# mirams/PyHillFit

Hardware: AMD Instinct MI355X
Metric: MCMC samples/sec (whole node) (higher is better)
Workload: dtype f64

## Files before the change

### pyhillfit_amd/csrc/phf_model.h

```cpp
#ifndef PHF_MODEL_H
#define PHF_MODEL_H

#include "phf_math.h"
#include "phf_philox.h"

#define PHF_SIGMA_FLOOR 1e-3
#define PHF_PIC50_RATE 0.2
#define PHF_PIC50_LOWER (-3.0)
#define PHF_HILL_UPPER 10.0
#define PHF_SIGMA_LOC 1e-3
#define PHF_SIGMA_SHAPE_M1 4.0
#define PHF_SIGMA_INV_SCALE (4.0 / (6.0 - 1e-3))
#define PHF_HILL_ARG_CAP 40.0

PHF_HD double phf_hill_den(int model, double ln_conc, double hill, double ln_ic50, phf_ktab k_exp) {
  const double a = (model == 1) ? (ln_conc - ln_ic50) : hill * (ln_conc - ln_ic50);
  return 1.0 + phf_exp_capped_k(__builtin_fmin(a, PHF_HILL_ARG_CAP), k_exp);
}

PHF_HD double phf_hill_percent(double w, phf_ktab k_exp) { return phf_fma(-PHF_K100(k_exp), w, PHF_K100(k_exp)); }
#define PHF_PCT_(w_) phf_hill_percent((w_), k_exp)

PHF_HD double phf_censored_z(double pred, double y, double inv_s) {
  const double sgn = (y > 50.0) ? 1.0 : -1.0;
  return (sgn * (pred - y)) * inv_s;
}

PHF_HD void phf_sl_log_target(int model, const double* lc, const double* y, const double* w, int n_other, int n_cens,
                              double n_other_points, double ss_within, double pi_bit, double temperature,
                              const double* th, phf_ktab k_exp, phf_ktab k_log,
                              double* out_lik, double* out_prior, double* out_ll1) {
  const double pic50 = th[0];
  const double hill = (model == 1) ? 1.0 : th[1];
  const double sigma = (model == 1) ? th[1] : th[2];
  const double ln_ic50 = PHF_LN10 * (6.0 - pic50);
  const double sl = sigma - PHF_SIGMA_LOC;
  const double inv_s = phf_rcp(sigma);
  const double log_sigma = phf_log_pos_k(sigma, k_log);
  const double log_sl = phf_log_pos_k(sl, k_log);

  double sse = ss_within, cens = 0.0;
  int j = 0;
  for (; j + 4 <= n_other; j += 4) {
    const phf_ktab ke = k_exp;
    const double d0 = phf_hill_den(model, lc[j], hill, ln_ic50, ke), d1 = phf_hill_den(model, lc[j + 1], hill, ln_ic50, ke);
    const double d2 = phf_hill_den(model, lc[j + 2], hill, ln_ic50, ke), d3 = phf_hill_den(model, lc[j + 3], hill, ln_ic50, ke);
    const double p01 = d0 * d1, p23 = d2 * d3;
    const double inv = phf_rcp(p01 * p23);
    const double i01 = inv * p23, i23 = inv * p01;
    const double r0 = y[j] - PHF_PCT_(i01 * d1), r1 = y[j + 1] - PHF_PCT_(i01 * d0);
    const double r2 = y[j + 2] - PHF_PCT_(i23 * d3), r3 = y[j + 3] - PHF_PCT_(i23 * d2);
    sse = phf_fma(w[j] * r0, r0, sse); sse = phf_fma(w[j + 1] * r1, r1, sse);
    sse = phf_fma(w[j + 2] * r2, r2, sse); sse = phf_fma(w[j + 3] * r3, r3, sse);
  }
  const int rem = n_other - j;
  if (rem == 3) {
    const phf_ktab ke = k_exp;
    const double d0 = phf_hill_den(model, lc[j], hill, ln_ic50, ke), d1 = phf_hill_den(model, lc[j + 1], hill, ln_ic50, ke);
    const double d2 = phf_hill_den(model, lc[j + 2], hill, ln_ic50, ke);
    const double p01 = d0 * d1;
    const double inv = phf_rcp(p01 * d2);
    const double i01 = inv * d2;
    const double r0 = y[j] - PHF_PCT_(i01 * d1), r1 = y[j + 1] - PHF_PCT_(i01 * d0);
    const double r2 = y[j + 2] - PHF_PCT_(inv * p01);
    sse = phf_fma(w[j] * r0, r0, sse); sse = phf_fma(w[j + 1] * r1, r1, sse); sse = phf_fma(w[j + 2] * r2, r2, sse);
  } else if (rem == 2) {
    const phf_ktab ke = k_exp;
    const double d0 = phf_hill_den(model, lc[j], hill, ln_ic50, ke), d1 = phf_hill_den(model, lc[j + 1], hill, ln_ic50, ke);
    const double inv = phf_rcp(d0 * d1);
    const double r0 = y[j] - PHF_PCT_(inv * d1), r1 = y[j + 1] - PHF_PCT_(inv * d0);
    sse = phf_fma(w[j] * r0, r0, sse); sse = phf_fma(w[j + 1] * r1, r1, sse);
  } else if (rem == 1) {
    const double r = y[j] - PHF_PCT_(phf_rcp(phf_hill_den(model, lc[j], hill, ln_ic50, k_exp)));
    sse = phf_fma(w[j] * r, r, sse);
  }
  j = n_other;
  const int n = n_other + n_cens;
  for (; j + 2 <= n; j += 2) {
    const phf_ktab ke = k_exp;
    const double d0 = phf_hill_den(model, lc[j], hill, ln_ic50, ke), d1 = phf_hill_den(model, lc[j + 1], hill, ln_ic50, ke);
    const double inv = phf_rcp(d0 * d1);
    const double z0 = phf_censored_z(PHF_PCT_(inv * d1), y[j], inv_s);
    const double z1 = phf_censored_z(PHF_PCT_(inv * d0), y[j + 1], inv_s);
    cens = phf_fma(w[j], phf_log_ndtr_tab(z0, -z0 * PHF_INV_SQRT2), cens);
    cens = phf_fma(w[j + 1], phf_log_ndtr_tab(z1, -z1 * PHF_INV_SQRT2), cens);
  }
  for (; j < n; ++j) {
    const double pred = PHF_PCT_(phf_rcp(phf_hill_den(model, lc[j], hill, ln_ic50, k_exp)));
    const double z = phf_censored_z(pred, y[j], inv_s);
    cens = phf_fma(w[j], phf_log_ndtr_tab(z, -z * PHF_INV_SQRT2), cens);
  }
  double a = cens - pi_bit;
  a = phf_fma(-n_other_points, log_sigma, a);
  a = phf_fma(-sse, 0.5 * inv_s * inv_s, a);
  if (sigma <= PHF_SIGMA_FLOOR) a = -PHF_INF;
  double lik = temperature * a;
  if (temperature == 0.0) lik = 0.0;
  *out_lik = lik;
  *out_ll1 = a;

  const int outside = (pic50 < PHF_PIC50_LOWER)
                      | (sigma <= PHF_SIGMA_LOC)
                      | ((model == 2) & ((hill < 0.0) | (hill > PHF_HILL_UPPER)));
  const double g = phf_fma(PHF_SIGMA_SHAPE_M1, log_sl, -sl * PHF_SIGMA_INV_SCALE);
  const double lp = -PHF_PIC50_RATE * pic50 + g;
  *out_prior = outside ? -PHF_INF : lp;
}

#define PHF_SHARE_PUT_(jj, d_) do { if (share_mask) den_slot[(jj) * slot_stride] = (d_); } while (0)
#define PHF_CDEN_(jj) ((((share_mask) >> ((jj) - n_other)) & 1u) ? den_slot[den_off[(jj) - n_other]] \
                                                                 : phf_hill_den(model, lc[jj], hill, ln_ic50, k_exp))
PHF_HD void phf_sl_log_target_shared(int model, const double* lc, const double* y, const double* w, int n_other, int n_cens,
                                     double n_other_points, double ss_within, double pi_bit, double temperature,
                                     const double* th, phf_ktab k_exp, phf_ktab k_log,
                                     unsigned share_mask, const int* den_off, double* den_slot, int slot_stride,
                                     double* out_lik, double* out_prior, double* out_ll1) {
  const double pic50 = th[0];
  const double hill = (model == 1) ? 1.0 : th[1];
  const double sigma = (model == 1) ? th[1] : th[2];
  const double ln_ic50 = PHF_LN10 * (6.0 - pic50);
  const double sl = sigma - PHF_SIGMA_LOC;
  const double inv_s = phf_rcp(sigma);
  const double log_sigma = phf_log_pos_k(sigma, k_log);
  const double log_sl = phf_log_pos_k(sl, k_log);

  double sse = ss_within, cens = 0.0;
  int j = 0;
  for (; j + 4 <= n_other; j += 4) {
    const phf_ktab ke = k_exp;
    const double d0 = phf_hill_den(model, lc[j], hill, ln_ic50, ke), d1 = phf_hill_den(model, lc[j + 1], hill, ln_ic50, ke);
    const double d2 = phf_hill_den(model, lc[j + 2], hill, ln_ic50, ke), d3 = phf_hill_den(model, lc[j + 3], hill, ln_ic50, ke);
    PHF_SHARE_PUT_(j, d0); PHF_SHARE_PUT_(j + 1, d1); PHF_SHARE_PUT_(j + 2, d2); PHF_SHARE_PUT_(j + 3, d3);
    const double p01 = d0 * d1, p23 = d2 * d3;
    const double inv = phf_rcp(p01 * p23);
    const double i01 = inv * p23, i23 = inv * p01;
    const double r0 = y[j] - PHF_PCT_(i01 * d1), r1 = y[j + 1] - PHF_PCT_(i01 * d0);
    const double r2 = y[j + 2] - PHF_PCT_(i23 * d3), r3 = y[j + 3] - PHF_PCT_(i23 * d2);
    sse = phf_fma(w[j] * r0, r0, sse); sse = phf_fma(w[j + 1] * r1, r1, sse);
    sse = phf_fma(w[j + 2] * r2, r2, sse); sse = phf_fma(w[j + 3] * r3, r3, sse);
  }
  const int rem = n_other - j;
  if (rem == 3) {
    const phf_ktab ke = k_exp;
    const double d0 = phf_hill_den(model, lc[j], hill, ln_ic50, ke), d1 = phf_hill_den(model, lc[j + 1], hill, ln_ic50, ke);
    const double d2 = phf_hill_den(model, lc[j + 2], hill, ln_ic50, ke);
    PHF_SHARE_PUT_(j, d0); PHF_SHARE_PUT_(j + 1, d1); PHF_SHARE_PUT_(j + 2, d2);
    const double p01 = d0 * d1;
    const double inv = phf_rcp(p01 * d2);
    const double i01 = inv * d2;
    const double r0 = y[j] - PHF_PCT_(i01 * d1), r1 = y[j + 1] - PHF_PCT_(i01 * d0);
    const double r2 = y[j + 2] - PHF_PCT_(inv * p01);
    sse = phf_fma(w[j] * r0, r0, sse); sse = phf_fma(w[j + 1] * r1, r1, sse); sse = phf_fma(w[j + 2] * r2, r2, sse);
  } else if (rem == 2) {
    const phf_ktab ke = k_exp;
    const double d0 = phf_hill_den(model, lc[j], hill, ln_ic50, ke), d1 = phf_hill_den(model, lc[j + 1], hill, ln_ic50, ke);
    PHF_SHARE_PUT_(j, d0); PHF_SHARE_PUT_(j + 1, d1);
    const double inv = phf_rcp(d0 * d1);
    const double r0 = y[j] - PHF_PCT_(inv * d1), r1 = y[j + 1] - PHF_PCT_(inv * d0);
    sse = phf_fma(w[j] * r0, r0, sse); sse = phf_fma(w[j + 1] * r1, r1, sse);
  } else if (rem == 1) {
    const double d0 = phf_hill_den(model, lc[j], hill, ln_ic50, k_exp);
    PHF_SHARE_PUT_(j, d0);
    const double r = y[j] - PHF_PCT_(phf_rcp(d0));
    sse = phf_fma(w[j] * r, r, sse);
  }
  j = n_other;
  const int n = n_other + n_cens;
  for (; j + 2 <= n; j += 2) {
    const double d0 = PHF_CDEN_(j), d1 = PHF_CDEN_(j + 1);
    const double inv = phf_rcp(d0 * d1);
    const double z0 = phf_censored_z(PHF_PCT_(inv * d1), y[j], inv_s);
    const double z1 = phf_censored_z(PHF_PCT_(inv * d0), y[j + 1], inv_s);
    cens = phf_fma(w[j], phf_log_ndtr_tab(z0, -z0 * PHF_INV_SQRT2), cens);
    cens = phf_fma(w[j + 1], phf_log_ndtr_tab(z1, -z1 * PHF_INV_SQRT2), cens);
  }
  for (; j < n; ++j) {
    const double pred = PHF_PCT_(phf_rcp(PHF_CDEN_(j)));
    const double z = phf_censored_z(pred, y[j], inv_s);
    cens = phf_fma(w[j], phf_log_ndtr_tab(z, -z * PHF_INV_SQRT2), cens);
  }
  double a = cens - pi_bit;
  a = phf_fma(-n_other_points, log_sigma, a);
  a = phf_fma(-sse, 0.5 * inv_s * inv_s, a);
  if (sigma <= PHF_SIGMA_FLOOR) a = -PHF_INF;
  double lik = temperature * a;
  if (temperature == 0.0) lik = 0.0;
  *out_lik = lik;
  *out_ll1 = a;

  const int outside = (pic50 < PHF_PIC50_LOWER)
                      | (sigma <= PHF_SIGMA_LOC)
                      | ((model == 2) & ((hill < 0.0) | (hill > PHF_HILL_UPPER)));
  const double g = phf_fma(PHF_SIGMA_SHAPE_M1, log_sl, -sl * PHF_SIGMA_INV_SCALE);
  const double lp = -PHF_PIC50_RATE * pic50 + g;
  *out_prior = outside ? -PHF_INF : lp;
}
#undef PHF_SHARE_PUT_
#undef PHF_CDEN_

PHF_HD double phf_sl_log_prior(int model, const double* th, phf_ktab k_log) {
  const double pic50 = th[0];
  const double hill = (model == 1) ? 1.0 : th[1];
  const double sigma = (model == 1) ? th[1] : th[2];
  const double sl = sigma - PHF_SIGMA_LOC;
  const double log_sl = phf_log_pos_k(sl, k_log);
  const int outside = (pic50 < PHF_PIC50_LOWER)
                      | (sigma <= PHF_SIGMA_LOC)
                      | ((model == 2) & ((hill < 0.0) | (hill > PHF_HILL_UPPER)));
  const double g = phf_fma(PHF_SIGMA_SHAPE_M1, log_sl, -sl * PHF_SIGMA_INV_SCALE);
  const double lp = -PHF_PIC50_RATE * pic50 + g;
  return outside ? -PHF_INF : lp;
}

PHF_HD double phf_mh_draws(int d, uint32_t chain_id, uint32_t problem_id, uint32_t t, uint32_t seed_lo,
                           uint32_t seed_hi, phf_ktab k_log, double* z) {
  const phf_u32x4 b = phf_philox_mh(chain_id, problem_id, t, 0u, seed_lo, seed_hi);
  z[0] = phf_normal_u32(b.w[0]);
  z[1] = phf_normal_u32(b.w[1]);
  if (d == 2) {
    z[2] = 0.0;
    const double u = phf_uniform53(b.w[2], b.w[3]);
    const double log_u = phf_log_pos_k(u, k_log);
    return (u < PHF_DBL_MIN) ? -PHF_INF : log_u;
  }
  z[2] = phf_normal_u32(b.w[2]);
  return phf_log_pos_k(phf_unit_open32(b.w[3]), k_log);
}

PHF_HD uint32_t phf_mh_draws_w3(uint32_t chain_id, uint32_t problem_id, uint32_t t, uint32_t seed_lo, uint32_t seed_hi, double* z) {
  const phf_u32x4 b = phf_philox_mh(chain_id, problem_id, t, 0u, seed_lo, seed_hi);
  z[0] = phf_normal_u32(b.w[0]);
  z[1] = phf_normal_u32(b.w[1]);
  z[2] = phf_normal_u32(b.w[2]);
  return b.w[3];
}

#define PHF_ACCEPT_U32_BAND 0x1p18f
PHF_HD int phf_mh_accept_u32(double x, uint32_t w, phf_ktab k_log) {
#if defined(__HIP_DEVICE_COMPILE__)
  const float t = __builtin_amdgcn_exp2f(__builtin_fmaf((float)x, 0x1.715476p+0f, 32.0f));
  const float dw = (float)w - t;
  bool acc = dw < 0.0f;
  if (PHF_ANY_LANE(__builtin_fabsf(dw) <= PHF_ACCEPT_U32_BAND)) {
    const bool exact = phf_log_pos_k(phf_unit_open32(w), k_log) < x;
    acc = (__builtin_fabsf(dw) <= PHF_ACCEPT_U32_BAND) ? exact : acc;
  }
  return acc;
#else
  return phf_log_pos_k(phf_unit_open32(w), k_log) < x;
#endif
}

#endif
```

### pyhillfit_amd/csrc/phf_philox.h

```cpp
#ifndef PHF_PHILOX_H
#define PHF_PHILOX_H

#include <stdint.h>

#if defined(__HIPCC__)
#define PHF_PHILOX_HD static __host__ __device__ __forceinline__
#else
#define PHF_PHILOX_HD static inline
#endif

typedef struct { uint32_t w[4]; } phf_u32x4;

#if defined(__HIP_DEVICE_COMPILE__)
#define PHF_XOR3(a, b, c) ((uint32_t)__builtin_amdgcn_bitop3_b32((int)(a), (int)(b), (int)(c), 0x96))
#else
#define PHF_XOR3(a, b, c) ((a) ^ (b) ^ (c))
#endif

#ifndef PHF_PHILOX_ROUNDS
#define PHF_PHILOX_ROUNDS 7
#endif

PHF_PHILOX_HD phf_u32x4 phf_philox4x32_r(int rounds, uint32_t c0, uint32_t c1, uint32_t c2, uint32_t c3,
                                         uint32_t k0, uint32_t k1) {
#if defined(__HIPCC__)
#pragma unroll
#endif
  for (int round = 0; round < rounds; ++round) {
    const uint64_t p0 = (uint64_t)0xD2511F53u * c0;
    const uint64_t p1 = (uint64_t)0xCD9E8D57u * c2;
    const uint32_t n0 = PHF_XOR3((uint32_t)(p1 >> 32), c1, k0);
    const uint32_t n2 = PHF_XOR3((uint32_t)(p0 >> 32), c3, k1);
    c1 = (uint32_t)p1; c3 = (uint32_t)p0; c0 = n0; c2 = n2;
    k0 += 0x9E3779B9u; k1 += 0xBB67AE85u;
  }
  phf_u32x4 out;
  out.w[0] = c0; out.w[1] = c1; out.w[2] = c2; out.w[3] = c3;
  return out;
}

PHF_PHILOX_HD phf_u32x4 phf_philox4x32_10(uint32_t c0, uint32_t c1, uint32_t c2, uint32_t c3, uint32_t k0, uint32_t k1) {
  return phf_philox4x32_r(10, c0, c1, c2, c3, k0, k1);
}
PHF_PHILOX_HD phf_u32x4 phf_philox4x32_7(uint32_t c0, uint32_t c1, uint32_t c2, uint32_t c3, uint32_t k0, uint32_t k1) {
  return phf_philox4x32_r(7, c0, c1, c2, c3, k0, k1);
}
PHF_PHILOX_HD phf_u32x4 phf_philox_mh(uint32_t c0, uint32_t c1, uint32_t c2, uint32_t c3, uint32_t k0, uint32_t k1) {
  return phf_philox4x32_r(PHF_PHILOX_ROUNDS, c0, c1, c2, c3, k0, k1);
}

#endif
```

### pyhillfit_amd/csrc/phf_single_level.hip

```cpp
#include <hip/hip_runtime.h>

#include "../../include/pyhillfit_amd.h"
#include "phf_common.h"
#include "phf_hier3_isa.h"
#include "phf_model.h"

namespace {

constexpr int kBlock = 64;
thread_local int g_last_sl_kernel = 0;
constexpr int kQueuePoison = 0x40000000;
constexpr int kQueueMaxRounds = 16;
constexpr int kDenSlots = 4;
constexpr int kMaxShared = 4;

template <int MODEL> struct Dim { static constexpr int d = (MODEL == 1) ? 2 : 3; };

#ifndef PHF_CHOL_FUSED_PIVOT
#define PHF_CHOL_FUSED_PIVOT 1
#endif
template <int D>
__device__ __forceinline__ void chol_packed(const double* c, double* l) {
  double inv[D];
#pragma unroll
  for (int i = 0; i < D; ++i) {
#pragma unroll
    for (int j = 0; j <= i; ++j) {
      double s = c[i * (i + 1) / 2 + j];
#pragma unroll
      for (int k = 0; k < j; ++k) s = phf_fma(-l[i * (i + 1) / 2 + k], l[j * (j + 1) / 2 + k], s);
      if (i == j) {
        const bool pos = s > 0.0;
        double ir = 0.0;
#if PHF_CHOL_FUSED_PIVOT
        const double rs = (i + 1 < D) ? phf_sqrt_rcp_pos(s, &ir) : phf_sqrt_pos(s);
#else
        const double rs = phf_sqrt_pos(s);
        ir = phf_rcp(rs);
#endif
        const double r = pos ? rs : 0.0;
        l[i * (i + 1) / 2 + i] = r;
        inv[i] = pos ? ir : 0.0;
      } else {
        l[i * (i + 1) / 2 + j] = s * inv[j];
      }
    }
  }
}

struct AdvanceArgs {
  phf_points pts;
  phf_problems prob;
  phf_mh_config cfg;
  int64_t t_begin, t_end;
  double* state;
  double* rows;
  double* moments;
  int64_t moments_after;
  int32_t blocks_per_problem;
  int32_t* queue;
  int32_t quantum;
  int32_t steady;
};

__device__ __forceinline__ void stage_points(const phf_points& pts, int pair, double* s_pts, int& n_other,
                                             int& n_zero, int& n_hundred) {
  const int32_t* cnt = pts.counts + 4 * pair;
  n_other = cnt[0]; n_zero = cnt[1]; n_hundred = cnt[2];
  const int n = n_other + n_zero + n_hundred;
  for (int j = threadIdx.x; j < n; j += kBlock) {
    s_pts[j] = pts.ln_conc[(size_t)pair * pts.stride + j];
    s_pts[pts.stride + j] = pts.response[(size_t)pair * pts.stride + j];
    s_pts[2 * pts.stride + j] = pts.weight[(size_t)pair * pts.stride + j];
  }
  __syncthreads();
}

template <int MODEL, bool MOMENTS, int KO, int KC, unsigned SHARE, bool LONE_WAVE, bool STEADY>
__device__ __forceinline__ void advance_body(const AdvanceArgs& a, const double* s_pts, double* s_den, const int* den_off, int q,
                                             int c, int pair, int n_other_rt, int n_cens_rt, const int64_t t_begin, const int64_t t_end) {
  static_assert(SHARE == 0 || (KO >= 1 && KO <= kDenSlots && KC >= 1 && KC <= kMaxShared && (SHARE >> KC) == 0),
                "shared denominators need a straight-line body with at most kDenSlots uncensored entries");
  constexpr int D = Dim<MODEL>::d;
  constexpr int NTRI = D * (D + 1) / 2;
  const int C = a.prob.chains_per_problem;
  const int n_other = (KO >= 0) ? KO : n_other_rt;
  const int n_cens = (KC >= 0) ? KC : n_cens_rt;
  const double* lc = s_pts;
  const double* yv = s_pts + a.pts.stride;
  const double* wv = s_pts + 2 * a.pts.stride;
  const double pi_bit = a.pts.pi_bit[pair];
  const double n_other_points = a.pts.extra[2 * pair], ss_within = a.pts.extra[2 * pair + 1];
  const double temperature = a.prob.temperature[q];
  const uint32_t pid = a.prob.problem_id[q];
  const uint32_t cid = a.prob.chain_id_base + (a.prob.chain_offset ? a.prob.chain_offset[q] : 0u) + (uint32_t)c;
  uint32_t seed_lo = (uint32_t)a.cfg.seed, seed_hi = (uint32_t)(a.cfg.seed >> 32);
  if (!LONE_WAVE) { asm volatile("" : "+v"(seed_lo)); asm volatile("" : "+v"(seed_hi)); }
  const size_t nchains = (size_t)a.prob.num_problems * C;
  const size_t g = (size_t)q * C + c;

  double th[D], mean[D], cov[NTRI], L[NTRI];
  double* sp = a.state + g;
#pragma unroll
  for (int i = 0; i < D; ++i) th[i] = sp[(size_t)i * nchains];
  double lt = sp[(size_t)D * nchains];
#pragma unroll
  for (int i = 0; i < D; ++i) mean[i] = sp[(size_t)(D + 1 + i) * nchains];
#pragma unroll
  for (int i = 0; i < NTRI; ++i) cov[i] = sp[(size_t)(2 * D + 1 + i) * nchains];
  double loga = sp[(size_t)(2 * D + 1 + NTRI) * nchains];
  const double nacc_in = sp[(size_t)(2 * D + 2 + NTRI) * nchains];
  uint32_t nacc = 0;
  double ll1 = sp[(size_t)(2 * D + 3 + NTRI) * nchains];
  PHF_KFETCH_V(k_exp, phf_k_exp, PHF_K_EXP_N);
  PHF_KFETCH_V(k_log, phf_k_log, PHF_K_LOG_N);
  chol_packed<D>(cov, L);
  double sc = phf_exp_fast_k(0.5 * loga, k_exp);

  double m1[D + 1], m2[D + 1], mll = 0.0;
  constexpr bool want_moments = MOMENTS;
  if (want_moments) {
#pragma unroll
    for (int i = 0; i <= D; ++i) {
      m1[i] = a.moments[(size_t)i * nchains + g];
      m2[i] = a.moments[(size_t)(D + 1 + i) * nchains + g];
    }
    mll = a.moments[(size_t)(2 * D + 2) * nchains + g];
  }

  const int thin = a.cfg.thinning;
  int until_save = thin - (int)(t_begin % thin);
  const bool save_rows = a.rows != nullptr;
  const size_t row_stride = (size_t)a.prob.num_problems * (D + 1) * C;
  double* out = a.rows + ((size_t)q * (D + 1)) * C + c + (size_t)(t_begin / thin - a.t_begin / thin) * row_stride;

  double z[3];
  double log_u = 0.0;
  uint32_t w_u = 0u;
  if constexpr (D == 3) w_u = phf_mh_draws_w3(cid, pid, (uint32_t)(t_begin + 1), seed_lo, seed_hi, z);
  else log_u = phf_mh_draws(D, cid, pid, (uint32_t)(t_begin + 1), seed_lo, seed_hi, k_log, z);
  const int64_t adapt_start = a.cfg.adapt_start;
  const bool adapt_in_range = adapt_start >= 0 && adapt_start <= 0xffffffffLL;
  const bool adapt_always = adapt_start < 0;
  const uint32_t adapt_at = adapt_start > 0xffffffffLL ? 0xffffffffu : (uint32_t)adapt_start;
  const bool reset_mean = a.cfg.reset_mean_at_adapt_start != 0 && adapt_in_range;
  const bool moments_always = a.moments_after < 0;
  const uint32_t moments_at = a.moments_after > 0xffffffffLL ? 0xffffffffu : (uint32_t)a.moments_after;
  int64_t gamma_i = t_begin + 1 - adapt_start;
  uint32_t t = (uint32_t)t_begin + 1u;
  for (uint32_t left = (uint32_t)(t_end - t_begin); left != 0; --left, ++t, ++gamma_i) {
    double star[D];
#pragma unroll
    for (int i = 0; i < D; ++i) {
      double v = L[i * (i + 1) / 2 + i] * z[i];
#pragma unroll
      for (int k = i - 1; k >= 0; --k) v = phf_fma(L[i * (i + 1) / 2 + k], z[k], v);
      star[i] = phf_fma(sc, v, th[i]);
    }
    double lik_star, prior_star, ll1_star;
    phf_sl_log_target_shared(MODEL, lc, yv, wv, n_other, n_cens, n_other_points, ss_within, pi_bit, temperature, star, k_exp, k_log,
                             SHARE, den_off, s_den + threadIdx.x, kBlock, &lik_star, &prior_star, &ll1_star);
    const double lt_star = lik_star + prior_star;
    const bool acc = (D == 3) ? (bool)phf_mh_accept_u32(lt_star - lt, w_u, k_log) : log_u < lt_star - lt;
    if (acc) {
#pragma unroll
      for (int i = 0; i < D; ++i) th[i] = star[i];
      lt = lt_star;
      ll1 = ll1_star;
    }
    nacc += acc ? 1u : 0u;
    double gs, gm, omg, omm;
    if constexpr (STEADY) {
      gs = a.cfg.gamma[gamma_i];
      omg = 1.0 - gs;
      gm = gs; omm = omg;
    } else {
      const bool adapting = adapt_always || t > adapt_at;
      const bool reset_now = reset_mean && t == adapt_at;
      const double gs_tab = a.cfg.gamma[adapting ? gamma_i : 0];
      gs = adapting ? gs_tab : 0.0;
      omg = 1.0 - gs;
      gm = reset_now ? 1.0 : gs; omm = reset_now ? 0.0 : omg;
    }
    {
      double v[D];
#pragma unroll
      for (int i = 0; i < D; ++i) v[i] = th[i] - mean[i];
#pragma unroll
      for (int i = 0; i < D; ++i)
#pragma unroll
        for (int j = 0; j <= i; ++j)
          cov[i * (i + 1) / 2 + j] = phf_fma(gs, v[i] * v[j], omg * cov[i * (i + 1) / 2 + j]);
#pragma unroll
      for (int i = 0; i < D; ++i) mean[i] = phf_fma(gm, th[i], omm * mean[i]);
      loga = phf_fma(gs, acc ? 0.75 : -0.25, loga);
    }
    double z_next[3];
    double log_u_next = 0.0;
    uint32_t w_u_next = 0u;
    if constexpr (D == 3) w_u_next = phf_mh_draws_w3(cid, pid, t + 1u, seed_lo, seed_hi, z_next);
    else log_u_next = phf_mh_draws(D, cid, pid, t + 1u, seed_lo, seed_hi, k_log, z_next);
    chol_packed<D>(cov, L);
    sc = phf_exp_fast_k(0.5 * loga, k_exp);
#pragma unroll
    for (int i = 0; i < 3; ++i) z[i] = z_next[i];
    log_u = log_u_next;
    w_u = w_u_next;
    if (--until_save == 0) {
      until_save = thin;
      if (save_rows) {
#pragma unroll
        for (int i = 0; i < D; ++i) out[(size_t)i * C] = th[i];
        out[(size_t)D * C] = lt;
        out += row_stride;
      }
      if (want_moments && (moments_always || t > moments_at)) {
#pragma unroll
        for (int i = 0; i < D; ++i) { m1[i] += th[i]; m2[i] = phf_fma(th[i], th[i], m2[i]); }
        m1[D] += lt; m2[D] = phf_fma(lt, lt, m2[D]);
        mll += ll1;
      }
    }
  }

#pragma unroll
  for (int i = 0; i < D; ++i) sp[(size_t)i * nchains] = th[i];
  sp[(size_t)D * nchains] = lt;
#pragma unroll
  for (int i = 0; i < D; ++i) sp[(size_t)(D + 1 + i) * nchains] = mean[i];
#pragma unroll
  for (int i = 0; i < NTRI; ++i) sp[(size_t)(2 * D + 1 + i) * nchains] = cov[i];
  sp[(size_t)(2 * D + 1 + NTRI) * nchains] = loga;
  sp[(size_t)(2 * D + 2 + NTRI) * nchains] = nacc_in + (double)nacc;
  sp[(size_t)(2 * D + 3 + NTRI) * nchains] = ll1;
  if (want_moments) {
#pragma unroll
    for (int i = 0; i <= D; ++i) {
      a.moments[(size_t)i * nchains + g] = m1[i];
      a.moments[(size_t)(D + 1 + i) * nchains + g] = m2[i];
    }
    a.moments[(size_t)(2 * D + 2) * nchains + g] = mll;
  }
}

#define PHF_BODY_(ko, kc, sh, steady) \
  advance_body<MODEL, MOMENTS, ko, kc, sh, WPS == 1, steady>(a, s_pts, s_den, den_off, q, c, pair, n_other, n_cens, t_from, t_to)
#define PHF_SHAPE_CASE(ko, kc) case (ko) * 8 + (kc): PHF_BODY_(ko, kc, 0u, true); break;
#define PHF_SHAPE_CASE_SHARED(ko, kc, sh) \
  case (ko) * 8 + (kc): if ((share & (sh)) == (sh)) PHF_BODY_(ko, kc, sh, true); else PHF_BODY_(ko, kc, 0u, true); break;
#define PHF_SHAPE_ROW(ko) PHF_SHAPE_CASE(ko, 0) PHF_SHAPE_CASE(ko, 1) PHF_SHAPE_CASE(ko, 2) PHF_SHAPE_CASE(ko, 3) PHF_SHAPE_CASE(ko, 4)

__device__ __forceinline__ unsigned share_map(const double* s_pts, int n_other, int n_cens, int* den_off) {
  unsigned share = 0;
#pragma unroll
  for (int m = 0; m < kMaxShared; ++m) {
    den_off[m] = 0;
    if (m < n_cens && n_other <= kDenSlots) {
      const long long b = __double_as_longlong(s_pts[n_other + m]);
#pragma unroll
      for (int j = kDenSlots - 1; j >= 0; --j)
        if (j < n_other && __double_as_longlong(s_pts[j]) == b) { share |= 1u << m; den_off[m] = j * kBlock; }
    }
    den_off[m] = __builtin_amdgcn_readfirstlane(den_off[m]);
  }
  return __builtin_amdgcn_readfirstlane(share);
}

template <int MODEL, bool MOMENTS, int WPS>
__device__ __forceinline__ void run_block(const AdvanceArgs& a, double* s_pts, double* s_den, int block, const int64_t t_begin,
                                          const int64_t t_end) {
  const int slot = block / a.blocks_per_problem;
  const int chunk = block - slot * a.blocks_per_problem;
  const int q = a.prob.launch_order ? a.prob.launch_order[slot] : slot;
  const int c = chunk * kBlock + threadIdx.x;
  int n_other, n_zero, n_hundred;
  const int pair = a.prob.pair_index[q];
  stage_points(a.pts, pair, s_pts, n_other, n_zero, n_hundred);
  if (c >= a.prob.chains_per_problem) return;
  const int n_cens = n_zero + n_hundred;
  int den_off[kMaxShared];
  const unsigned share = share_map(s_pts, n_other, n_cens, den_off);
  int64_t t_from = t_begin, t_to = t_end;
  if (a.steady == 0 || t_begin < a.cfg.adapt_start) {
    if (a.steady != 0 && a.cfg.adapt_start < t_end) t_to = a.cfg.adapt_start;
    PHF_BODY_(-1, -1, 0u, false);
    if (t_to == t_end) return;
    t_from = t_to; t_to = t_end;
  }
  if (n_other <= 5 && n_cens <= 4) {
    switch (n_other * 8 + n_cens) {
      PHF_SHAPE_CASE(0, 1) PHF_SHAPE_CASE(0, 2) PHF_SHAPE_CASE(0, 3) PHF_SHAPE_CASE(0, 4)
      PHF_SHAPE_CASE(1, 0) PHF_SHAPE_CASE(1, 1) PHF_SHAPE_CASE(1, 2) PHF_SHAPE_CASE(1, 3) PHF_SHAPE_CASE_SHARED(1, 4, 0x8u)
      PHF_SHAPE_CASE(2, 0) PHF_SHAPE_CASE_SHARED(2, 1, 0x1u) PHF_SHAPE_CASE_SHARED(2, 2, 0x3u) PHF_SHAPE_CASE_SHARED(2, 3, 0x4u)
      PHF_SHAPE_CASE_SHARED(2, 4, 0xcu)
      PHF_SHAPE_CASE(3, 0) PHF_SHAPE_CASE(3, 1) PHF_SHAPE_CASE_SHARED(3, 2, 0x2u) PHF_SHAPE_CASE_SHARED(3, 3, 0x6u)
      PHF_SHAPE_CASE_SHARED(3, 4, 0xeu)
      PHF_SHAPE_CASE(4, 0) PHF_SHAPE_CASE_SHARED(4, 1, 0x1u) PHF_SHAPE_CASE_SHARED(4, 2, 0x3u) PHF_SHAPE_CASE_SHARED(4, 3, 0x7u)
      PHF_SHAPE_CASE_SHARED(4, 4, 0xfu)
      PHF_SHAPE_ROW(5)
      default: PHF_BODY_(-1, -1, 0u, true); break;
    }
    return;
  }
  PHF_BODY_(-1, -1, 0u, true);
}

template <int MODEL, bool MOMENTS, int WPS>
__global__ __launch_bounds__(kBlock, WPS) void mh_advance_kernel(const AdvanceArgs a) {
  PHF_MATH_TABLES_TO_LDS();
  PHF_NORMAL_TABLE_TO_LDS();
  PHF_LOGPHI_TABLE_TO_LDS();
  extern __shared__ double s_pts[];
  __shared__ double s_den[kDenSlots * kBlock];
  const bool queued = a.queue != nullptr;
  const int nblocks = a.blocks_per_problem * a.prob.num_problems;
  const int total = queued ? nblocks * (int)((a.t_end - a.t_begin + a.quantum - 1) / a.quantum) : 0;
  for (;;) {
    int b = blockIdx.x, k = 0;
    int64_t t0 = a.t_begin, t1 = a.t_end;
    if (queued) {
      int task = 0;
      if (threadIdx.x == 0) task = atomicAdd(a.queue, 1);
      task = __builtin_amdgcn_readfirstlane(task);
      if (task >= total) break;
      k = task / nblocks; b = task - k * nblocks;
      if (k > 0) {
        int polls = 0;
        while (__hip_atomic_load(a.queue + 1 + b, __ATOMIC_RELAXED, __HIP_MEMORY_SCOPE_AGENT) < k) {
          __builtin_amdgcn_s_sleep(16);
          ++polls;
          const bool gave_up = polls > (1 << 24) ||
                               ((polls & 1023) == 0 && __hip_atomic_load(a.queue + 1 + nblocks, __ATOMIC_RELAXED, __HIP_MEMORY_SCOPE_AGENT) != 0);
          if (gave_up) {
            if (threadIdx.x == 0) {
              __hip_atomic_store(a.queue + 1 + nblocks, 1, __ATOMIC_RELAXED, __HIP_MEMORY_SCOPE_AGENT);
              __hip_atomic_store(a.queue, kQueuePoison, __ATOMIC_RELAXED, __HIP_MEMORY_SCOPE_AGENT);
            }
            return;
          }
        }
        __builtin_amdgcn_fence(__ATOMIC_ACQUIRE, "agent");
      }
      t0 = a.t_begin + (int64_t)k * a.quantum;
      t1 = (t0 + a.quantum < a.t_end) ? t0 + a.quantum : a.t_end;
    }
    run_block<MODEL, MOMENTS, WPS>(a, s_pts, s_den, b, t0, t1);
    if (!queued) break;
    __builtin_amdgcn_fence(__ATOMIC_RELEASE, "agent");
    asm volatile("s_waitcnt vmcnt(0)" ::: "memory");
    __syncthreads();
    if (threadIdx.x == 0) __hip_atomic_store(a.queue + 1 + b, k + 1, __ATOMIC_RELAXED, __HIP_MEMORY_SCOPE_AGENT);
  }
}

struct InitArgs {
  phf_points pts;
  phf_problems prob;
  int32_t cov_identity;
  double cov_scale;
  const double* theta0;
  double* state;
  double* row0;
  int32_t blocks_per_problem;
};

template <int MODEL>
__global__ __launch_bounds__(kBlock) void mh_init_kernel(const InitArgs a) {
  PHF_MATH_TABLES_TO_LDS();
  PHF_LOGPHI_TABLE_TO_LDS();
  constexpr int D = Dim<MODEL>::d;
  constexpr int NTRI = D * (D + 1) / 2;
  extern __shared__ double s_pts[];
  const int q = blockIdx.x / a.blocks_per_problem;
  const int chunk = blockIdx.x - q * a.blocks_per_problem;
  const int C = a.prob.chains_per_problem;
  const int c = chunk * kBlock + threadIdx.x;
  int n_other, n_zero, n_hundred;
  const int pair = a.prob.pair_index[q];
  stage_points(a.pts, pair, s_pts, n_other, n_zero, n_hundred);
  if (c >= C) return;
  const size_t nchains = (size_t)a.prob.num_problems * C;
  const size_t g = (size_t)q * C + c;
  double th[D];
#pragma unroll
  for (int i = 0; i < D; ++i) th[i] = a.theta0[(size_t)i * nchains + g];
  double lik0, prior0, ll10;
  PHF_KFETCH_V(k_exp, phf_k_exp, PHF_K_EXP_N);
  PHF_KFETCH_V(k_log, phf_k_log, PHF_K_LOG_N);
  phf_sl_log_target(MODEL, s_pts, s_pts + a.pts.stride, s_pts + 2 * a.pts.stride, n_other, n_zero + n_hundred,
                    a.pts.extra[2 * pair], a.pts.extra[2 * pair + 1], a.pts.pi_bit[pair], a.prob.temperature[q],
                    th, k_exp, k_log, &lik0, &prior0, &ll10);
  const double lt = lik0 + prior0;
  double* sp = a.state + g;
#pragma unroll
  for (int i = 0; i < D; ++i) { sp[(size_t)i * nchains] = th[i]; sp[(size_t)(D + 1 + i) * nchains] = th[i]; }
  sp[(size_t)D * nchains] = lt;
#pragma unroll
  for (int i = 0; i < D; ++i)
#pragma unroll
    for (int j = 0; j <= i; ++j)
      sp[(size_t)(2 * D + 1 + i * (i + 1) / 2 + j) * nchains] =
          (i != j) ? 0.0 : (a.cov_identity ? a.cov_scale : a.cov_scale * __builtin_fabs(th[i]));
  sp[(size_t)(2 * D + 1 + NTRI) * nchains] = 0.0;
  sp[(size_t)(2 * D + 2 + NTRI) * nchains] = 0.0;
  sp[(size_t)(2 * D + 3 + NTRI) * nchains] = ll10;
  if (a.row0) {
    double* o = a.row0 + ((size_t)q * (D + 1)) * C + c;
#pragma unroll
    for (int i = 0; i < D; ++i) o[(size_t)i * C] = th[i];
    o[(size_t)D * C] = lt;
  }
}

template <int MODEL>
__global__ __launch_bounds__(256) void log_target_kernel(const phf_points pts, int64_t m, const int32_t* pair_index,
                                                          const double* temperature, const double* theta,
                                                          double* out_lik, double* out_prior) {
  PHF_MATH_TABLES_TO_LDS();
  PHF_LOGPHI_TABLE_TO_LDS();
  constexpr int D = Dim<MODEL>::d;
  const int64_t i = (int64_t)blockIdx.x * 256 + threadIdx.x;
  if (i >= m) return;
  const int pair = pair_index[i];
  const int32_t* cnt = pts.counts + 4 * pair;
  double th[D];
#pragma unroll
  for (int k = 0; k < D; ++k) th[k] = theta[(size_t)k * m + i];
  double lik, prior, ll1;
  PHF_KFETCH_V(k_exp, phf_k_exp, PHF_K_EXP_N);
  PHF_KFETCH_V(k_log, phf_k_log, PHF_K_LOG_N);
  phf_sl_log_target(MODEL, pts.ln_conc + (size_t)pair * pts.stride, pts.response + (size_t)pair * pts.stride,
                    pts.weight + (size_t)pair * pts.stride, cnt[0], cnt[1] + cnt[2], pts.extra[2 * pair], pts.extra[2 * pair + 1],
                    pts.pi_bit[pair], temperature[i], th, k_exp, k_log, &lik, &prior, &ll1);
  if (out_lik) out_lik[i] = lik;
  if (out_prior) out_prior[i] = prior;
}

__global__ void debug_math_kernel(int fn, int64_t n, const double* in, double* out) {
  PHF_MATH_TABLES_TO_LDS();
  PHF_LOGPHI_TABLE_TO_LDS();
  PHF_ERFC_TABLE_TO_LDS();
  PHF_NORMAL_TABLE_TO_LDS();
// ... 227 lines not shown
```

Baseline: 73.47 billion.

## Split Philox rounds into lane-invariant and wave-uniform parts; drop redundant sigma floor

Precomputes the first two Philox rounds' per-chain (lane) contributions once, and computes the per-iteration part that depends only on problem id and step with wave-uniform (readfirstlane) values. Each step then only runs the remaining rounds, which cuts per-step VALU integer multiplies in the RNG. It also removes the likelihood's sigma floor check in the MH path, because the prior already returns -inf at the same bound (enforced by a static_assert). This relies on pid and t being wave-uniform and on the algebraic split exactly reproducing the original Philox stream.

```diff
diff --git a/pyhillfit_amd/csrc/phf_model.h b/pyhillfit_amd/csrc/phf_model.h
--- a/pyhillfit_amd/csrc/phf_model.h
+++ b/pyhillfit_amd/csrc/phf_model.h
@@ -110,11 +110,12 @@
 #define PHF_SHARE_PUT_(jj, d_) do { if (share_mask) den_slot[(jj) * slot_stride] = (d_); } while (0)
 #define PHF_CDEN_(jj) ((((share_mask) >> ((jj) - n_other)) & 1u) ? den_slot[den_off[(jj) - n_other]] \
                                                                  : phf_hill_den(model, lc[jj], hill, ln_ic50, k_exp))
-PHF_HD void phf_sl_log_target_shared(int model, const double* lc, const double* y, const double* w, int n_other, int n_cens,
-                                     double n_other_points, double ss_within, double pi_bit, double temperature,
-                                     const double* th, phf_ktab k_exp, phf_ktab k_log,
-                                     unsigned share_mask, const int* den_off, double* den_slot, int slot_stride,
-                                     double* out_lik, double* out_prior, double* out_ll1) {
+PHF_HD void phf_sl_log_target_shared_impl_(int model, const double* lc, const double* y, const double* w, int n_other, int n_cens,
+                                           double n_other_points, double ss_within, double pi_bit, double temperature,
+                                           const double* th, phf_ktab k_exp, phf_ktab k_log,
+                                           unsigned share_mask, const int* den_off, double* den_slot, int slot_stride,
+                                           int floor_select,
+                                           double* out_lik, double* out_prior, double* out_ll1) {
   const double pic50 = th[0];
   const double hill = (model == 1) ? 1.0 : th[1];
   const double sigma = (model == 1) ? th[1] : th[2];
@@ -182,7 +183,7 @@
   double a = cens - pi_bit;
   a = phf_fma(-n_other_points, log_sigma, a);
   a = phf_fma(-sse, 0.5 * inv_s * inv_s, a);
-  if (sigma <= PHF_SIGMA_FLOOR) a = -PHF_INF;
+  if (floor_select && sigma <= PHF_SIGMA_FLOOR) a = -PHF_INF;
   double lik = temperature * a;
   if (temperature == 0.0) lik = 0.0;
   *out_lik = lik;
@@ -197,6 +198,29 @@
 }
 #undef PHF_SHARE_PUT_
 #undef PHF_CDEN_
+
+PHF_HD void phf_sl_log_target_shared(int model, const double* lc, const double* y, const double* w, int n_other, int n_cens,
+                                     double n_other_points, double ss_within, double pi_bit, double temperature,
+                                     const double* th, phf_ktab k_exp, phf_ktab k_log,
+                                     unsigned share_mask, const int* den_off, double* den_slot, int slot_stride,
+                                     double* out_lik, double* out_prior, double* out_ll1) {
+  phf_sl_log_target_shared_impl_(model, lc, y, w, n_other, n_cens, n_other_points, ss_within, pi_bit, temperature, th, k_exp, k_log,
+                                 share_mask, den_off, den_slot, slot_stride, 1, out_lik, out_prior, out_ll1);
+}
+
+#if defined(__cplusplus)
+static_assert(PHF_SIGMA_FLOOR == PHF_SIGMA_LOC, "phf_sl_log_target_shared_mh: the floor of the likelihood must be the prior's support bound");
+#else
+_Static_assert(PHF_SIGMA_FLOOR == PHF_SIGMA_LOC, "phf_sl_log_target_shared_mh: the floor of the likelihood must be the prior's support bound");
+#endif
+PHF_HD void phf_sl_log_target_shared_mh(int model, const double* lc, const double* y, const double* w, int n_other, int n_cens,
+                                        double n_other_points, double ss_within, double pi_bit, double temperature,
+                                        const double* th, phf_ktab k_exp, phf_ktab k_log,
+                                        unsigned share_mask, const int* den_off, double* den_slot, int slot_stride,
+                                        double* out_lik, double* out_prior, double* out_ll1) {
+  phf_sl_log_target_shared_impl_(model, lc, y, w, n_other, n_cens, n_other_points, ss_within, pi_bit, temperature, th, k_exp, k_log,
+                                 share_mask, den_off, den_slot, slot_stride, 0, out_lik, out_prior, out_ll1);
+}
 
 PHF_HD double phf_sl_log_prior(int model, const double* th, phf_ktab k_log) {
   const double pic50 = th[0];
@@ -212,9 +236,7 @@
   return outside ? -PHF_INF : lp;
 }
 
-PHF_HD double phf_mh_draws(int d, uint32_t chain_id, uint32_t problem_id, uint32_t t, uint32_t seed_lo,
-                           uint32_t seed_hi, phf_ktab k_log, double* z) {
-  const phf_u32x4 b = phf_philox_mh(chain_id, problem_id, t, 0u, seed_lo, seed_hi);
+PHF_HD double phf_mh_draws_block(int d, phf_u32x4 b, phf_ktab k_log, double* z) {
   z[0] = phf_normal_u32(b.w[0]);
   z[1] = phf_normal_u32(b.w[1]);
   if (d == 2) {
@@ -226,13 +248,21 @@
   z[2] = phf_normal_u32(b.w[2]);
   return phf_log_pos_k(phf_unit_open32(b.w[3]), k_log);
 }
-
-PHF_HD uint32_t phf_mh_draws_w3(uint32_t chain_id, uint32_t problem_id, uint32_t t, uint32_t seed_lo, uint32_t seed_hi, double* z) {
+PHF_HD double phf_mh_draws(int d, uint32_t chain_id, uint32_t problem_id, uint32_t t, uint32_t seed_lo,
+                           uint32_t seed_hi, phf_ktab k_log, double* z) {
   const phf_u32x4 b = phf_philox_mh(chain_id, problem_id, t, 0u, seed_lo, seed_hi);
+  return phf_mh_draws_block(d, b, k_log, z);
+}
+
+PHF_HD uint32_t phf_mh_draws_w3_block(phf_u32x4 b, double* z) {
   z[0] = phf_normal_u32(b.w[0]);
   z[1] = phf_normal_u32(b.w[1]);
   z[2] = phf_normal_u32(b.w[2]);
   return b.w[3];
+}
+PHF_HD uint32_t phf_mh_draws_w3(uint32_t chain_id, uint32_t problem_id, uint32_t t, uint32_t seed_lo, uint32_t seed_hi, double* z) {
+  const phf_u32x4 b = phf_philox_mh(chain_id, problem_id, t, 0u, seed_lo, seed_hi);
+  return phf_mh_draws_w3_block(b, z);
 }
 
 #define PHF_ACCEPT_U32_BAND 0x1p18f
diff --git a/pyhillfit_amd/csrc/phf_philox.h b/pyhillfit_amd/csrc/phf_philox.h
--- a/pyhillfit_amd/csrc/phf_philox.h
+++ b/pyhillfit_amd/csrc/phf_philox.h
@@ -49,4 +49,51 @@
   return phf_philox4x32_r(PHF_PHILOX_ROUNDS, c0, c1, c2, c3, k0, k1);
 }
 
+typedef struct { uint32_t a, b, c1; } phf_philox_lane;
+typedef struct { uint32_t a, b, c3; } phf_philox_wave;
+
+PHF_PHILOX_HD phf_philox_lane phf_philox_split_lane(uint32_t c0, uint32_t k0, uint32_t k1) {
+  const uint64_t p0 = (uint64_t)0xD2511F53u * c0;
+  const uint32_t n2 = (uint32_t)(p0 >> 32) ^ k1;
+  const uint64_t q1 = (uint64_t)0xCD9E8D57u * n2;
+  phf_philox_lane l;
+  l.a = (uint32_t)(q1 >> 32) ^ (k0 + 0x9E3779B9u);
+  l.b = (uint32_t)p0 ^ (k1 + 0xBB67AE85u);
+  l.c1 = (uint32_t)q1;
+  return l;
+}
+
+PHF_PHILOX_HD phf_philox_wave phf_philox_split_wave(uint32_t c1, uint32_t c2, uint32_t k0) {
+  const uint64_t p1 = (uint64_t)0xCD9E8D57u * c2;
+  const uint32_t n0 = (uint32_t)(p1 >> 32) ^ c1 ^ k0;
+  const uint64_t q0 = (uint64_t)0xD2511F53u * n0;
+  phf_philox_wave w;
+  w.a = (uint32_t)p1;
+  w.b = (uint32_t)(q0 >> 32);
+  w.c3 = (uint32_t)q0;
+  return w;
+}
+
+PHF_PHILOX_HD phf_u32x4 phf_philox_split_join(int rounds, phf_philox_lane l, phf_philox_wave w, uint32_t k0, uint32_t k1) {
+  uint32_t c0 = l.a ^ w.a, c1 = l.c1, c2 = l.b ^ w.b, c3 = w.c3;
+  k0 += 2u * 0x9E3779B9u; k1 += 2u * 0xBB67AE85u;
+#if defined(__HIPCC__)
+#pragma unroll
 #endif
+  for (int round = 2; round < rounds; ++round) {
+    const uint64_t p0 = (uint64_t)0xD2511F53u * c0;
+    const uint64_t p1 = (uint64_t)0xCD9E8D57u * c2;
+    const uint32_t n0 = PHF_XOR3((uint32_t)(p1 >> 32), c1, k0);
+    const uint32_t n2 = PHF_XOR3((uint32_t)(p0 >> 32), c3, k1);
+    c1 = (uint32_t)p1; c3 = (uint32_t)p0; c0 = n0; c2 = n2;
+    k0 += 0x9E3779B9u; k1 += 0xBB67AE85u;
+  }
+  phf_u32x4 out;
+  out.w[0] = c0; out.w[1] = c1; out.w[2] = c2; out.w[3] = c3;
+  return out;
+}
+PHF_PHILOX_HD phf_u32x4 phf_philox_mh_join(phf_philox_lane l, phf_philox_wave w, uint32_t k0, uint32_t k1) {
+  return phf_philox_split_join(PHF_PHILOX_ROUNDS, l, w, k0, k1);
+}
+
+#endif
diff --git a/pyhillfit_amd/csrc/phf_single_level.hip b/pyhillfit_amd/csrc/phf_single_level.hip
--- a/pyhillfit_amd/csrc/phf_single_level.hip
+++ b/pyhillfit_amd/csrc/phf_single_level.hip
@@ -18,6 +18,12 @@
 
 #ifndef PHF_CHOL_FUSED_PIVOT
 #define PHF_CHOL_FUSED_PIVOT 1
+#endif
+#ifndef PHF_SL_PHILOX_SPLIT
+#define PHF_SL_PHILOX_SPLIT 1
+#endif
+#ifndef PHF_SL_MH_NO_FLOOR
+#define PHF_SL_MH_NO_FLOOR 1
 #endif
 template <int D>
 __device__ __forceinline__ void chol_packed(const double* c, double* l) {
@@ -96,6 +102,17 @@
   const uint32_t cid = a.prob.chain_id_base + (a.prob.chain_offset ? a.prob.chain_offset[q] : 0u) + (uint32_t)c;
   uint32_t seed_lo = (uint32_t)a.cfg.seed, seed_hi = (uint32_t)(a.cfg.seed >> 32);
   if (!LONE_WAVE) { asm volatile("" : "+v"(seed_lo)); asm volatile("" : "+v"(seed_hi)); }
+#if PHF_SL_PHILOX_SPLIT
+  const uint32_t pid_s = __builtin_amdgcn_readfirstlane(pid);
+  const uint32_t k0_s = __builtin_amdgcn_readfirstlane((uint32_t)a.cfg.seed);
+  const phf_philox_lane ph_lane = phf_philox_split_lane(cid, seed_lo, seed_hi);
+#define PHF_SL_BLOCK_(t_) phf_philox_mh_join(ph_lane, phf_philox_split_wave(pid_s, __builtin_amdgcn_readfirstlane(t_), k0_s), seed_lo, seed_hi)
+#define PHF_SL_DRAWS_W3_(t_, z_) phf_mh_draws_w3_block(PHF_SL_BLOCK_(t_), z_)
+#define PHF_SL_DRAWS_(t_, z_) phf_mh_draws_block(D, PHF_SL_BLOCK_(t_), k_log, z_)
+#else
+#define PHF_SL_DRAWS_W3_(t_, z_) phf_mh_draws_w3(cid, pid, t_, seed_lo, seed_hi, z_)
+#define PHF_SL_DRAWS_(t_, z_) phf_mh_draws(D, cid, pid, t_, seed_lo, seed_hi, k_log, z_)
+#endif
   const size_t nchains = (size_t)a.prob.num_problems * C;
   const size_t g = (size_t)q * C + c;
 
@@ -137,8 +154,8 @@
   double z[3];
   double log_u = 0.0;
   uint32_t w_u = 0u;
-  if constexpr (D == 3) w_u = phf_mh_draws_w3(cid, pid, (uint32_t)(t_begin + 1), seed_lo, seed_hi, z);
-  else log_u = phf_mh_draws(D, cid, pid, (uint32_t)(t_begin + 1), seed_lo, seed_hi, k_log, z);
+  if constexpr (D == 3) w_u = PHF_SL_DRAWS_W3_((uint32_t)(t_begin + 1), z);
+  else log_u = PHF_SL_DRAWS_((uint32_t)(t_begin + 1), z);
   const int64_t adapt_start = a.cfg.adapt_start;
   const bool adapt_in_range = adapt_start >= 0 && adapt_start <= 0xffffffffLL;
   const bool adapt_always = adapt_start < 0;
@@ -158,8 +175,13 @@
       star[i] = phf_fma(sc, v, th[i]);
     }
     double lik_star, prior_star, ll1_star;
+#if PHF_SL_MH_NO_FLOOR
+    phf_sl_log_target_shared_mh(MODEL, lc, yv, wv, n_other, n_cens, n_other_points, ss_within, pi_bit, temperature, star, k_exp, k_log,
+                                SHARE, den_off, s_den + threadIdx.x, kBlock, &lik_star, &prior_star, &ll1_star);
+#else
     phf_sl_log_target_shared(MODEL, lc, yv, wv, n_other, n_cens, n_other_points, ss_within, pi_bit, temperature, star, k_exp, k_log,
                              SHARE, den_off, s_den + threadIdx.x, kBlock, &lik_star, &prior_star, &ll1_star);
+#endif
     const double lt_star = lik_star + prior_star;
     const bool acc = (D == 3) ? (bool)phf_mh_accept_u32(lt_star - lt, w_u, k_log) : log_u < lt_star - lt;
     if (acc) {
@@ -198,8 +220,8 @@
     double z_next[3];
     double log_u_next = 0.0;
     uint32_t w_u_next = 0u;
-    if constexpr (D == 3) w_u_next = phf_mh_draws_w3(cid, pid, t + 1u, seed_lo, seed_hi, z_next);
-    else log_u_next = phf_mh_draws(D, cid, pid, t + 1u, seed_lo, seed_hi, k_log, z_next);
+    if constexpr (D == 3) w_u_next = PHF_SL_DRAWS_W3_(t + 1u, z_next);
+    else log_u_next = PHF_SL_DRAWS_(t + 1u, z_next);
     chol_packed<D>(cov, L);
     sc = phf_exp_fast_k(0.5 * loga, k_exp);
 #pragma unroll
@@ -241,6 +263,9 @@
     }
     a.moments[(size_t)(2 * D + 2) * nchains + g] = mll;
   }
+#undef PHF_SL_BLOCK_
+#undef PHF_SL_DRAWS_W3_
+#undef PHF_SL_DRAWS_
 }
 
 #define PHF_BODY_(ko, kc, sh, steady) \
```

New measurement: 73.99 billion, median of 6. About the same (+0.7%).

## Add steady-state sampler target with unclamped exp, deferred outside test, fast Cholesky

Applied to the files above, without the earlier changes.

Adds a steady-phase log-target that computes the Hill exponential without its lower clamp when every dose is bounded below. It returns the prior-outside flag separately so the -inf selects are folded into the accept decision. The steady loop also uses a Cholesky without per-pivot positivity selects, falling back to the guarded version only when some lane sees a non-positive pivot. A per-problem check on dose bounds gates the specialized shape cases, which adds kernel code and a fallback branch.

```diff
diff --git a/pyhillfit_amd/csrc/phf_model.h b/pyhillfit_amd/csrc/phf_model.h
--- a/pyhillfit_amd/csrc/phf_model.h
+++ b/pyhillfit_amd/csrc/phf_model.h
@@ -195,6 +195,105 @@
   const double lp = -PHF_PIC50_RATE * pic50 + g;
   *out_prior = outside ? -PHF_INF : lp;
 }
+
+#define PHF_LN_CONC_NOCLAMP (-50.0)
+#if defined(__cplusplus)
+static_assert(PHF_SIGMA_FLOOR == PHF_SIGMA_LOC, "sigma <= floor must imply outside");
+#else
+_Static_assert(PHF_SIGMA_FLOOR == PHF_SIGMA_LOC, "sigma <= floor must imply outside");
+#endif
+PHF_HD double phf_hill_den_sampler(int model, double ln_conc, double hill, double ln_ic50, int lower_clamp, phf_ktab k_exp) {
+  const double a = (model == 1) ? (ln_conc - ln_ic50) : hill * (ln_conc - ln_ic50);
+  const double c = __builtin_fmin(a, PHF_HILL_ARG_CAP);
+  return 1.0 + (lower_clamp ? phf_exp_capped_k(c, k_exp) : phf_exp_core_k(c, k_exp));
+}
+#define PHF_DEN_(jj) phf_hill_den_sampler(model, lc[jj], hill, ln_ic50, lower_clamp, k_exp)
+#define PHF_CDEN_S_(jj) ((((share_mask) >> ((jj) - n_other)) & 1u) ? den_slot[den_off[(jj) - n_other]] : PHF_DEN_(jj))
+PHF_HD int phf_sl_log_target_sampler(int model, const double* lc, const double* y, const double* w, int n_other, int n_cens,
+                                     double n_other_points, double ss_within, double pi_bit, double temperature, int lower_clamp,
+                                     const double* th, phf_ktab k_exp, phf_ktab k_log,
+                                     unsigned share_mask, const int* den_off, double* den_slot, int slot_stride,
+                                     double* out_lik, double* out_prior, double* out_ll1, double* out_lt) {
+  const double pic50 = th[0];
+  const double hill = (model == 1) ? 1.0 : th[1];
+  const double sigma = (model == 1) ? th[1] : th[2];
+  const double ln_ic50 = PHF_LN10 * (6.0 - pic50);
+  const double sl = sigma - PHF_SIGMA_LOC;
+  const double inv_s = phf_rcp(sigma);
+  const double log_sigma = phf_log_pos_k(sigma, k_log);
+  const double log_sl = phf_log_pos_k(sl, k_log);
+
+  double sse = ss_within, cens = 0.0;
+  int j = 0;
+  for (; j + 4 <= n_other; j += 4) {
+    const double d0 = PHF_DEN_(j), d1 = PHF_DEN_(j + 1);
+    const double d2 = PHF_DEN_(j + 2), d3 = PHF_DEN_(j + 3);
+    PHF_SHARE_PUT_(j, d0); PHF_SHARE_PUT_(j + 1, d1); PHF_SHARE_PUT_(j + 2, d2); PHF_SHARE_PUT_(j + 3, d3);
+    const double p01 = d0 * d1, p23 = d2 * d3;
+    const double inv = phf_rcp(p01 * p23);
+    const double i01 = inv * p23, i23 = inv * p01;
+    const double r0 = y[j] - PHF_PCT_(i01 * d1), r1 = y[j + 1] - PHF_PCT_(i01 * d0);
+    const double r2 = y[j + 2] - PHF_PCT_(i23 * d3), r3 = y[j + 3] - PHF_PCT_(i23 * d2);
+    sse = phf_fma(w[j] * r0, r0, sse); sse = phf_fma(w[j + 1] * r1, r1, sse);
+    sse = phf_fma(w[j + 2] * r2, r2, sse); sse = phf_fma(w[j + 3] * r3, r3, sse);
+  }
+  const int rem = n_other - j;
+  if (rem == 3) {
+    const double d0 = PHF_DEN_(j), d1 = PHF_DEN_(j + 1);
+    const double d2 = PHF_DEN_(j + 2);
+    PHF_SHARE_PUT_(j, d0); PHF_SHARE_PUT_(j + 1, d1); PHF_SHARE_PUT_(j + 2, d2);
+    const double p01 = d0 * d1;
+    const double inv = phf_rcp(p01 * d2);
+    const double i01 = inv * d2;
+    const double r0 = y[j] - PHF_PCT_(i01 * d1), r1 = y[j + 1] - PHF_PCT_(i01 * d0);
+    const double r2 = y[j + 2] - PHF_PCT_(inv * p01);
+    sse = phf_fma(w[j] * r0, r0, sse); sse = phf_fma(w[j + 1] * r1, r1, sse); sse = phf_fma(w[j + 2] * r2, r2, sse);
+  } else if (rem == 2) {
+    const double d0 = PHF_DEN_(j), d1 = PHF_DEN_(j + 1);
+    PHF_SHARE_PUT_(j, d0); PHF_SHARE_PUT_(j + 1, d1);
+    const double inv = phf_rcp(d0 * d1);
+    const double r0 = y[j] - PHF_PCT_(inv * d1), r1 = y[j + 1] - PHF_PCT_(inv * d0);
+    sse = phf_fma(w[j] * r0, r0, sse); sse = phf_fma(w[j + 1] * r1, r1, sse);
+  } else if (rem == 1) {
+    const double d0 = PHF_DEN_(j);
+    PHF_SHARE_PUT_(j, d0);
+    const double r = y[j] - PHF_PCT_(phf_rcp(d0));
+    sse = phf_fma(w[j] * r, r, sse);
+  }
+  j = n_other;
+  const int n = n_other + n_cens;
+  for (; j + 2 <= n; j += 2) {
+    const double d0 = PHF_CDEN_S_(j), d1 = PHF_CDEN_S_(j + 1);
+    const double inv = phf_rcp(d0 * d1);
+    const double z0 = phf_censored_z(PHF_PCT_(inv * d1), y[j], inv_s);
+    const double z1 = phf_censored_z(PHF_PCT_(inv * d0), y[j + 1], inv_s);
+    cens = phf_fma(w[j], phf_log_ndtr_tab(z0, -z0 * PHF_INV_SQRT2), cens);
+    cens = phf_fma(w[j + 1], phf_log_ndtr_tab(z1, -z1 * PHF_INV_SQRT2), cens);
+  }
+  for (; j < n; ++j) {
+    const double pred = PHF_PCT_(phf_rcp(PHF_CDEN_S_(j)));
+    const double z = phf_censored_z(pred, y[j], inv_s);
+    cens = phf_fma(w[j], phf_log_ndtr_tab(z, -z * PHF_INV_SQRT2), cens);
+  }
+  double a = cens - pi_bit;
+  a = phf_fma(-n_other_points, log_sigma, a);
+  a = phf_fma(-sse, 0.5 * inv_s * inv_s, a);
+  *out_ll1 = a;
+
+  const int outside = (pic50 < PHF_PIC50_LOWER)
+                      | (sigma <= PHF_SIGMA_LOC)
+                      | ((model == 2) & ((hill < 0.0) | (hill > PHF_HILL_UPPER)));
+  const double g = phf_fma(PHF_SIGMA_SHAPE_M1, log_sl, -sl * PHF_SIGMA_INV_SCALE);
+  const double lp = -PHF_PIC50_RATE * pic50 + g;
+  *out_prior = lp;
+  double lik = temperature * a;
+  if (temperature == 0.0) lik = 0.0;
+  *out_lik = lik;
+  *out_lt = lik + lp;
+  return outside;
+}
+#undef PHF_DEN_
+#undef PHF_CDEN_S_
 #undef PHF_SHARE_PUT_
 #undef PHF_CDEN_
 
diff --git a/pyhillfit_amd/csrc/phf_single_level.hip b/pyhillfit_amd/csrc/phf_single_level.hip
--- a/pyhillfit_amd/csrc/phf_single_level.hip
+++ b/pyhillfit_amd/csrc/phf_single_level.hip
@@ -48,6 +48,40 @@
   }
 }
 
+#ifndef PHF_SL_STEADY_CHOL
+#define PHF_SL_STEADY_CHOL 1
+#endif
+#ifndef PHF_SL_STEADY_NOCLAMP
+#define PHF_SL_STEADY_NOCLAMP 1
+#endif
+template <int D>
+__device__ __forceinline__ void chol_packed_steady(const double* c, double* l) {
+  double inv[D];
+  bool bad = false;
+#pragma unroll
+  for (int i = 0; i < D; ++i) {
+#pragma unroll
+    for (int j = 0; j <= i; ++j) {
+      double s = c[i * (i + 1) / 2 + j];
+#pragma unroll
+      for (int k = 0; k < j; ++k) s = phf_fma(-l[i * (i + 1) / 2 + k], l[j * (j + 1) / 2 + k], s);
+      if (i == j) {
+        bad |= !(s > 0.0);
+        inv[i] = 0.0;
+        l[i * (i + 1) / 2 + i] = (i + 1 < D) ? phf_sqrt_rcp_pos(s, &inv[i]) : phf_sqrt_pos(s);
+      } else {
+        l[i * (i + 1) / 2 + j] = s * inv[j];
+      }
+    }
+  }
+  if (PHF_ANY_LANE(bad)) {
+    double lg[D * (D + 1) / 2];
+    chol_packed<D>(c, lg);
+#pragma unroll
+    for (int i = 0; i < D * (D + 1) / 2; ++i) l[i] = bad ? lg[i] : l[i];
+  }
+}
+
 struct AdvanceArgs {
   phf_points pts;
   phf_problems prob;
@@ -83,6 +117,7 @@
                 "shared denominators need a straight-line body with at most kDenSlots uncensored entries");
   constexpr int D = Dim<MODEL>::d;
   constexpr int NTRI = D * (D + 1) / 2;
+  constexpr int kLowerClamp = !(PHF_SL_STEADY_NOCLAMP && STEADY && KO >= 0);
   const int C = a.prob.chains_per_problem;
   const int n_other = (KO >= 0) ? KO : n_other_rt;
   const int n_cens = (KC >= 0) ? KC : n_cens_rt;
@@ -157,18 +192,26 @@
       for (int k = i - 1; k >= 0; --k) v = phf_fma(L[i * (i + 1) / 2 + k], z[k], v);
       star[i] = phf_fma(sc, v, th[i]);
     }
-    double lik_star, prior_star, ll1_star;
-    phf_sl_log_target_shared(MODEL, lc, yv, wv, n_other, n_cens, n_other_points, ss_within, pi_bit, temperature, star, k_exp, k_log,
-                             SHARE, den_off, s_den + threadIdx.x, kBlock, &lik_star, &prior_star, &ll1_star);
-    const double lt_star = lik_star + prior_star;
-    const bool acc = (D == 3) ? (bool)phf_mh_accept_u32(lt_star - lt, w_u, k_log) : log_u < lt_star - lt;
+    double lik_star, prior_star, ll1_star, lt_star;
+    bool inside = true;
+    if constexpr (STEADY) {
+      inside = !phf_sl_log_target_sampler(MODEL, lc, yv, wv, n_other, n_cens, n_other_points, ss_within, pi_bit, temperature,
+                                          kLowerClamp, star, k_exp, k_log, SHARE, den_off, s_den + threadIdx.x, kBlock, &lik_star, &prior_star,
+                                          &ll1_star, &lt_star);
+    } else {
+      phf_sl_log_target_shared(MODEL, lc, yv, wv, n_other, n_cens, n_other_points, ss_within, pi_bit, temperature, star, k_exp, k_log,
+                               SHARE, den_off, s_den + threadIdx.x, kBlock, &lik_star, &prior_star, &ll1_star);
+      lt_star = lik_star + prior_star;
+    }
+    const bool acc = inside & ((D == 3) ? (bool)phf_mh_accept_u32(lt_star - lt, w_u, k_log) : log_u < lt_star - lt);
     if (acc) {
 #pragma unroll
       for (int i = 0; i < D; ++i) th[i] = star[i];
       lt = lt_star;
       ll1 = ll1_star;
-    }
-    nacc += acc ? 1u : 0u;
+      if constexpr (STEADY) ++nacc;
+    }
+    if constexpr (!STEADY) nacc += acc ? 1u : 0u;
     double gs, gm, omg, omm;
     if constexpr (STEADY) {
       gs = a.cfg.gamma[gamma_i];
@@ -200,7 +243,8 @@
     uint32_t w_u_next = 0u;
     if constexpr (D == 3) w_u_next = phf_mh_draws_w3(cid, pid, t + 1u, seed_lo, seed_hi, z_next);
     else log_u_next = phf_mh_draws(D, cid, pid, t + 1u, seed_lo, seed_hi, k_log, z_next);
-    chol_packed<D>(cov, L);
+    if constexpr (STEADY && PHF_SL_STEADY_CHOL) chol_packed_steady<D>(cov, L);
+    else chol_packed<D>(cov, L);
     sc = phf_exp_fast_k(0.5 * loga, k_exp);
 #pragma unroll
     for (int i = 0; i < 3; ++i) z[i] = z_next[i];
@@ -287,7 +331,12 @@
     if (t_to == t_end) return;
     t_from = t_to; t_to = t_end;
   }
-  if (n_other <= 5 && n_cens <= 4) {
+  int doses_bounded = 1;
+  if (PHF_SL_STEADY_NOCLAMP && n_other <= 5 && n_cens <= 4) {
+    for (int j = 0; j < n_other + n_cens; ++j) doses_bounded &= (int)(s_pts[j] >= PHF_LN_CONC_NOCLAMP);
+    doses_bounded = __builtin_amdgcn_readfirstlane(doses_bounded);
+  }
+  if (n_other <= 5 && n_cens <= 4 && doses_bounded) {
     switch (n_other * 8 + n_cens) {
       PHF_SHAPE_CASE(0, 1) PHF_SHAPE_CASE(0, 2) PHF_SHAPE_CASE(0, 3) PHF_SHAPE_CASE(0, 4)
       PHF_SHAPE_CASE(1, 0) PHF_SHAPE_CASE(1, 1) PHF_SHAPE_CASE(1, 2) PHF_SHAPE_CASE(1, 3) PHF_SHAPE_CASE_SHARED(1, 4, 0x8u)
```

Result: faster. 74.70 billion before, 76.15 billion after (median of 6 runs) (+1.9%).
